# cherise215/advchain

Hardware: AMD Instinct MI355X
Metric: augmented images/sec (N adv steps, chain=noise+bias+morph+affine) (higher is better)
Workload: dtype f32

## Files before the change

advchain_amd/_lib.py:

```python
import ctypes
import os
from ctypes import c_char_p, c_float, c_int, c_int64, c_void_p

_HERE = os.path.dirname(os.path.abspath(__file__))
LIB_PATH = os.path.join(_HERE, "csrc", "libadvchain_hip.so")

_P, _I, _L, _F = c_void_p, c_int, c_int64, c_float

PROTOTYPES = {
    "advchain_version": (_I, []),
    "advchain_last_error": (c_char_p, []),
    "advchain_set_deterministic": (None, [_I]),
    "advchain_get_deterministic": (_I, []),
    "advchain_grid_sample_fwd": (_I, [_P, _P, _P, _L, _L, _I, _P, _P, _I, _I, _I, _P]),
    "advchain_grid_sample_fwd_ride": (_I, [_P, _P, _P, _P, _P, _L, _L, _I, _P, _P, _I, _I, _I, _I, _P]),
    "advchain_scatter_workspace": (_L, [_L, _I, _P]),
    "advchain_grid_sample_bwd": (_I, [_P, _P, _P, _P, _P, _P, _L, _L, _I, _P, _P, _I, _I, _I, _I, _P]),
    "advchain_compose_self_fwd": (_I, [_P, _P, _P, _L, _I, _P, _I, _P, _P]),
    "advchain_compose_self_bwd": (_I, [_P, _P, _P, _P, _I, _I, _L, _I, _P, _P]),
    "advchain_affine_warp_fwd": (_I, [_P, _P, _P, _L, _L, _I, _P, _I, _I, _P]),
    "advchain_affine_warp_fwd_ride": (_I, [_P, _P, _P, _P, _P, _L, _L, _I, _P, _I, _I, _I, _P]),
    "advchain_affine_warp_bwd_workspace": (_L, [_L, _I, _P]),
    "advchain_affine_warp_bwd": (_I, [_P, _P, _P, _P, _P, _P, _L, _L, _I, _P, _I, _I, _P]),
    "advchain_affine_theta_fwd": (_I, [_P, _P, _F, _P, _P, _L, _I, _P]),
    "advchain_affine_theta_bwd": (_I, [_P, _P, _F, _P, _P, _P, _L, _I, _P]),
    "advchain_tp_interp_fwd": (_I, [_P, _P, _P, _P, _P, _P, _P, _L, _L, _I, _I, _F, _P, _P, _P]),
    "advchain_tp_interp_fwd_smoothed_pair": (_I, [_P, _P, _P, _P, _P, _P, _P, _P, _L, _L, _I, _F, _P, _P, _F, _P]),
    "advchain_band_reduce_axis": (_I, [_P, _P, _P, _P, _P, _P, _P, _P, _I, _L, _L, _F, _P]),
    "advchain_band_reduce_rows_dense": (_I, [_P, _P, _P, _P, _P, _L, _L, _L, _L, _F, _P]),
    "advchain_bias_field_fwd": (_I, [_P, _P, _P, _P, _P, _P, _P, _P, _P, _L, _L, _F, _I, _F, _P]),
    "advchain_bias_field_bwd": (_I, [_P, _P, _P, _P, _P, _P, _P, _P, _P, _P, _L, _L, _F, _I, _F, _P]),
    "advchain_gauss_axis": (_I, [_P, _P, _P, _L, _L, _I, _P, _I, _P, _I, _I, _F, _P]),
    "advchain_gauss_axis_generic": (_I, [_P, _P, _L, _I, _P, _I, _P, _I, _F, _P]),
    "advchain_max_displacement": (_I, [_P, _P, _L, _I, _P, _P]),
    "advchain_grid_sample_bicubic2d_fwd": (_I, [_P, _P, _P, _L, _L, _P, _P, _I, _P]),
    "advchain_grid_sample_bicubic2d_bwd": (_I, [_P, _P, _P, _P, _P, _L, _L, _P, _P, _I, _P]),
    "advchain_affine_grid2d_fwd": (_I, [_P, _P, _L, _P, _P]),
    "advchain_affine_grid2d_bwd_workspace": (_L, [_L, _P]),
    "advchain_affine_grid2d_bwd": (_I, [_P, _P, _P, _L, _P, _P]),
    "advchain_slot_rows_max": (_I, [_P, _P, _L, _L, _I, _P]),
    "advchain_demons_compose_pair_fwd": (_I, [_P, _P, _P, _P, _P, _P, _P, _P, _P, _P, _P, _P, _P, _L, _I, _I, _P, _P, _F, _F, _I, _P]),
    "advchain_demons_compose_pair_bwd": (_I, [_P, _P, _P, _P, _P, _P, _P, _P, _P, _P, _P, _P, _P, _P, _P, _P, _P, _L, _P, _P, _P, _L,
                                              _I, _I, _P, _F, _F, _P]),
    "advchain_bounds_check": (_I, [_P, _P, _P, _L, _P, _P]),
    "advchain_expo_chain_fused_levels": (_I, [_L, _I, _P, _I, _P]),
    "advchain_expo_chain_fwd": (_I, [_P, _P, _P, _L, _I, _P, _I, _P, _P, _P, _P]),
# ... 132 lines not shown
```

advchain_amd/csrc/error.cpp:

```cpp
#include <string.h>

#include <atomic>

static thread_local char g_last_error[512] = "";

extern "C" void advchain_set_error_(const char* msg) {
  strncpy(g_last_error, msg ? msg : "", sizeof(g_last_error) - 1);
  g_last_error[sizeof(g_last_error) - 1] = 0;
}

extern "C" const char* advchain_last_error(void) { return g_last_error; }

static std::atomic<int> g_deterministic{0};
extern "C" void advchain_set_deterministic(int on) { g_deterministic.store(on ? 1 : 0, std::memory_order_relaxed); }
extern "C" int advchain_get_deterministic(void) { return g_deterministic.load(std::memory_order_relaxed); }

extern "C" int advchain_version(void) { return 130; }
```

advchain_amd/csrc/sampler.hip:

```cpp
#include <stdlib.h>
#include "sampler_common.h"
#include "affine_geo.h"

namespace advchain {

template <int UNR>
__device__ __forceinline__ void load_str(const float* __restrict__ p, int n, float (&r)[UNR]) {
#pragma unroll
  for (int k = 0; k < UNR; ++k) r[k] = p[(k < n ? k : 0) * kBlock];
#pragma unroll
  for (int k = 0; k < UNR; ++k) r[k] = k < n ? r[k] : 0.f;
}
template <int UNR>
__device__ __forceinline__ void store_str(float* __restrict__ p, int n, const float (&r)[UNR]) {
#pragma unroll
  for (int k = 0; k < UNR; ++k)
    if (k < n) p[k * kBlock] = r[k];
}
__device__ __forceinline__ int active_count(int64_t v0, int64_t total, int unr) {
  if (v0 >= total) return 0;
  const int64_t left = (total - v0 + kBlock - 1) / kBlock;
  return left < unr ? (int)left : unr;
}

// ... 620 lines not shown
  const int row = blockIdx.x;
  const int k = blockIdx.y;
  __shared__ float smem[4];
  float s[1] = {0.f};
  for (int b = threadIdx.x; b < nb; b += blockDim.x) s[0] += partial[((int64_t)row * nb + b) * K + k];
  block_sum<1>(s, smem);
  if (threadIdx.x == 0) out[(int64_t)row * K + k] = s[0];
}

}

using namespace advchain;

int advchain_scatter_tiled_launch(bool self, const float* gout, const float* in, const float* grid, float* gin,
                                  float* ggrid, int64_t N, int64_t C, int ndim, Dims d, int padding, int clamp_grid,
                                  int32_t* workspace, int chain, int halo, hipStream_t st);

int advchain_self_adjoint_gather_launch(const float* gout, const float* phi, float* gphi, int64_t N, int ndim, Dims d,
                                        int32_t* workspace, int chain, int halo, hipStream_t st);

int advchain_warp_adjoint_gather_launch(const float* gout, const float* in, const float* grid, float* gin, float* ggrid,
                                        int64_t N, int64_t C, int ndim, Dims d, int padding, int clamp_grid,
                                        int32_t* workspace, int halo, hipStream_t st);

int advchain_scatter_march_launch(bool self, const float* gout, const float* in, const float* grid, float* gin, float* ggrid,
                                  int64_t N, int64_t C, Dims d, int padding, int clamp_grid, int H, int32_t* workspace,
                                  hipStream_t st);

int advchain_scatter_window_launch(bool self, const float* gout, const float* in, const float* grid, float* gin,
                                   float* ggrid, int64_t N, int64_t C, int ndim, Dims d, int padding, int clamp_grid,
                                   int halo, int32_t* workspace, hipStream_t st, int32_t* det_ws);
int advchain_scatter_rows2d_launch(bool self, const float* gout, const float* in, const float* grid, float* gin, float* ggrid,
                                   int64_t N, int64_t C, Dims d, int padding, int clamp_grid, int H, int32_t* workspace,
                                   hipStream_t st, int rm_flags = 0);
bool advchain_scatter_rows2d_takes(bool self, int64_t C, Dims d, int padding, int H, int64_t N);

bool advchain_affine_box_fwd_launch(const float* in, const float* theta, float* out, int64_t N, int64_t C, int ndim, Dims d,
                                    hipStream_t st, const float* ride_in = nullptr, float* ride_out = nullptr,
                                    int ride_nonzero = 0);
int advchain_affine_box_tiles(int ndim, Dims d);
int advchain_affine_box_gtheta_launch(const float* gout, const float* in, const float* theta, float* gpart, int64_t N,
                                      int64_t C, int ndim, Dims d, int max_blocks, hipStream_t st, float* tilemax, float* geo = nullptr, int* mode = nullptr);
bool advchain_affine_box_gin_launch(const float* gout, const float* theta, const float* geo, const int* mode, float* gin,
                                    int64_t N, int64_t C, int ndim, Dims d, hipStream_t st, const float* tilemax);

int advchain_expo_fused_fwd2d_launch(const float* phi0, float* fields, int64_t N, advchain::Dims d, int k, int halos,
                                     float* disp_rows, float* fail_flag, hipStream_t stream, bool query = false);
int advchain_adjoint_fused2d_launch(const float* gk, const float* phi0, const float* fields, float* g0, int64_t N, advchain::Dims d,
                                    int k, int32_t* workspace, hipStream_t st);
int advchain_sample_tiled_launch(bool self, const float* in, const float* grid, float* out, const float* phi0,
                                 int64_t N, int64_t C, int ndim, Dims d, int padding, int clamp_grid, int final_mode,
                                 int halo, float* disp_out, hipStream_t st, int disp_hint);

static inline bool use_unroll(int64_t voxels, int ndim) {
  static const bool force1 = false;
  static const bool force4 = false;
  if (force4) return true;
  return !force1 && ndim == 2 && voxels >= 4 * kBlock;
}

#define DISPATCH_PAD(PADV, ...)                                            \
  switch (PADV) {                                                          \
    case PAD_ZEROS: { constexpr int PAD = PAD_ZEROS; __VA_ARGS__; } break; \
    case PAD_BORDER: { constexpr int PAD = PAD_BORDER; __VA_ARGS__; } break; \
    default: { constexpr int PAD = PAD_REFLECTION; __VA_ARGS__; } break;   \
  }

// ... 167 lines not shown
  ADVCHAIN_CHECK_ARG(final_mode == 0 || (final_mode == 1 && phi0), "compose_self_fwd: final_mode 1 needs phi0");
  ADVCHAIN_CHECK_ARG(N >= 0 && N < 65536, "compose_self_fwd: bad N");
  if (N == 0) return ADVCHAIN_OK;
  const Dims d = make_dims(ndim, dims);
  const int64_t V = d.voxels();
  ADVCHAIN_CHECK_ARG(V < (1ll << 31), "compose_self_fwd: per-sample volume too large");
  {
    const int rc = advchain_sample_tiled_launch(true, phi, nullptr, out, phi0, N, ndim, ndim, d, PAD_BORDER, 0,
                                                final_mode, 0, disp_out, (hipStream_t)stream, disp_hint);
    if (rc != ADVCHAIN_ERR_UNSUPPORTED) return rc;
  }
  const bool vec4 = use_unroll(V, ndim);
  hipStream_t st = (hipStream_t)stream;
  static const bool unr2 = true && true;
  if (unr2 && vec4 && ndim == 2) {
    dim3 g2(advchain_blocks(V, kBlock * 2), (unsigned)N);
    hipLaunchKernelGGL((k_compose_self_fwd<2, 2>), g2, dim3(kBlock), 0, st, phi, out, phi0, d, final_mode, disp_out);
    ADVCHAIN_LAUNCH_CHECK();
    return ADVCHAIN_OK;
  }
  dim3 g(advchain_blocks(V, kBlock * (vec4 ? 4 : 1)), (unsigned)N), b(kBlock);
  if (ndim == 3) {
    if (vec4) hipLaunchKernelGGL((k_compose_self_fwd<3, 4>), g, b, 0, st, phi, out, phi0, d, final_mode, disp_out);
    else hipLaunchKernelGGL((k_compose_self_fwd<3, 1>), g, b, 0, st, phi, out, phi0, d, final_mode, disp_out);
  } else {
    if (vec4) hipLaunchKernelGGL((k_compose_self_fwd<2, 4>), g, b, 0, st, phi, out, phi0, d, final_mode, disp_out);
    else hipLaunchKernelGGL((k_compose_self_fwd<2, 1>), g, b, 0, st, phi, out, phi0, d, final_mode, disp_out);
  }
  ADVCHAIN_LAUNCH_CHECK();
  return ADVCHAIN_OK;
}

static int compose_self_bwd_impl(const float* grad_out, const float* phi, float* grad_phi, int32_t* workspace, int chain,
                                 int halo, int64_t N, int ndim, const int64_t* dims, void* stream, int rm_flags);

int advchain_compose_self_bwd(const float* grad_out, const float* phi, float* grad_phi, int32_t* workspace, int chain,
                              int halo, int64_t N, int ndim, const int64_t* dims, void* stream) {
  return compose_self_bwd_impl(grad_out, phi, grad_phi, workspace, chain, halo, N, ndim, dims, stream, 0);
}

static int compose_self_bwd_impl(const float* grad_out, const float* phi, float* grad_phi, int32_t* workspace, int chain,
                                 int halo, int64_t N, int ndim, const int64_t* dims, void* stream, int rm_flags) {
  ADVCHAIN_CHECK_ARG(grad_out && phi && grad_phi, "compose_self_bwd: null pointer");
  ADVCHAIN_CHECK_ARG(dims_ok(ndim, dims), "compose_self_bwd: bad dims");
  ADVCHAIN_CHECK_ARG(N >= 0 && N < 65536, "compose_self_bwd: bad N");
  if (N == 0) return ADVCHAIN_OK;
  const Dims d = make_dims(ndim, dims);
  const int64_t V = d.voxels();
  ADVCHAIN_CHECK_ARG(V < (1ll << 31), "compose_self_bwd: per-sample volume too large");
  if (workspace) {
    if (ndim == 2 && halo <= -2) {
      const int rr = advchain_scatter_rows2d_launch(true, grad_out, phi, phi, grad_phi, nullptr, N, ndim, d, PAD_BORDER, 0, -halo,
                                                    workspace, (hipStream_t)stream, rm_flags);
      if (rr != ADVCHAIN_ERR_UNSUPPORTED) return rr;
    }
    const int rc = advchain_self_adjoint_gather_launch(grad_out, phi, grad_phi, N, ndim, d, workspace, chain, halo,
                                                       (hipStream_t)stream);
    if (rc != ADVCHAIN_ERR_UNSUPPORTED) return rc;
    if (ndim == 3 && halo <= -2) {
      const int rm = advchain_scatter_march_launch(true, grad_out, phi, phi, grad_phi, nullptr, N, ndim, d, PAD_BORDER, 0, -halo,
                                                   workspace, (hipStream_t)stream);
      if (rm != ADVCHAIN_ERR_UNSUPPORTED) return rm;
    }
    const int rw = advchain_scatter_window_launch(true, grad_out, phi, phi, grad_phi, nullptr, N, ndim, ndim, d, PAD_BORDER,
                                                  0, halo, workspace, (hipStream_t)stream, workspace);
    if (rw != ADVCHAIN_ERR_UNSUPPORTED) return rw;
    return advchain_scatter_tiled_launch(true, grad_out, phi, phi, grad_phi, nullptr, N, ndim, ndim, d, PAD_BORDER, 0,
                                         workspace, chain, halo < 0 ? -halo : halo, (hipStream_t)stream);
  }
  const bool vec4 = use_unroll(V, ndim);
  dim3 g(advchain_blocks(V, kBlock * (vec4 ? 4 : 1)), (unsigned)N), b(kBlock);
  hipStream_t st = (hipStream_t)stream;
  if (ndim == 3) {
    if (vec4) hipLaunchKernelGGL((k_compose_self_bwd<3, 4>), g, b, 0, st, grad_out, phi, grad_phi, d);
    else hipLaunchKernelGGL((k_compose_self_bwd<3, 1>), g, b, 0, st, grad_out, phi, grad_phi, d);
  } else {
    if (vec4) hipLaunchKernelGGL((k_compose_self_bwd<2, 4>), g, b, 0, st, grad_out, phi, grad_phi, d);
    else hipLaunchKernelGGL((k_compose_self_bwd<2, 1>), g, b, 0, st, grad_out, phi, grad_phi, d);
  }
  ADVCHAIN_LAUNCH_CHECK();
  return ADVCHAIN_OK;
}

int advchain_affine_warp_fwd(const float* in, const float* theta, float* out, int64_t N, int64_t C, int ndim,
                             const int64_t* dims, int interp, int padding, void* stream) {
  ADVCHAIN_CHECK_ARG(in && theta && out, "affine_warp_fwd: null pointer");
// ... 128 lines not shown
    }
  }
  if (fused) src = fields + (int64_t)(fused - 1) * F;
  for (int m = fused; m + 1 < n; ++m) {
    float* dst = fields + (int64_t)m * F;
    const int rc = advchain_compose_self_fwd(src, dst, nullptr, N, ndim, dims, hints ? (hints[m] & 0xff) << 8 : 0,
                                             disp_rows ? disp_rows + (int64_t)(m + 1) * kDispSlots : nullptr, stream);
    if (rc != ADVCHAIN_OK) return rc;
    src = dst;
  }
  return advchain_compose_self_fwd(src, pos, phi0, N, ndim, dims, 1 | (hints ? (hints[n - 1] & 0xff) << 8 : 0),
                                   disp_rows ? disp_rows + (int64_t)n * kDispSlots : nullptr, stream);
}

int advchain_expo_chain_bwd(const float* grad_pos, const float* phi0, const float* fields, float* grad_phi0, float* scratch,
                            int32_t* workspace, const int32_t* halos, int64_t N, int ndim, const int64_t* dims, int n,
                            void* stream) {
  ADVCHAIN_CHECK_ARG(grad_pos && phi0 && grad_phi0 && n >= 1 && n <= 64 && (n == 1 || (fields && scratch)) && halos,
                     "expo_chain_bwd: null pointer / bad n");
  ADVCHAIN_CHECK_ARG(dims_ok(ndim, dims), "expo_chain_bwd: bad dims");
  ADVCHAIN_CHECK_ARG(grad_phi0 != scratch && grad_pos != grad_phi0 && grad_pos != scratch, "expo_chain_bwd: aliased buffers");
  const int64_t F = N * ndim * make_dims(ndim, dims).voxels();
  int kf = 0;
  if (ndim == 2 && workspace && n >= 2) {
    while (kf < n && kf < 4 && halos[n - 1 - kf] == -1) ++kf;
    if (kf < 2) kf = 0;
  }
  const float* g = grad_pos;
  const Dims dd = make_dims(ndim, dims);
  static const bool no_handover = getenv("ADVCHAIN_NO_ROWMAX_HANDOVER") != nullptr;
  auto rows = [&](int i) {
    return !no_handover && ndim == 2 && workspace && i >= 0 && i < n - kf && halos[i] <= -2 && advchain_scatter_rows2d_takes(true, 2, dd, PAD_BORDER, -halos[i], N);
  };
  for (int i = 0; i < n - kf; ++i) {
    const int m = n - 1 - i;
    const float* phi = m == 0 ? phi0 : fields + (int64_t)(m - 1) * F;
    float* out = ((m - kf) % 2 == 0) ? (kf ? scratch : grad_phi0) : (kf ? grad_phi0 : scratch);
    const int rm = rows(i) ? ((rows(i - 1) ? 1 : 0) | (rows(i + 1) ? 2 : 0) | ((i & 1) ? 4 : 0)) : 0;
    const int rc = compose_self_bwd_impl(g, phi, out, workspace, i > 0 ? 1 : 0, halos[i], N, ndim, dims, stream, rm);
    if (rc != ADVCHAIN_OK) return rc;
    g = out;
  }
  if (kf) {
    const int rf = advchain_adjoint_fused2d_launch(g, phi0, fields, grad_phi0, N, make_dims(ndim, dims), kf, workspace,
                                                   (hipStream_t)stream);
    if (rf == ADVCHAIN_ERR_UNSUPPORTED) {
      for (int m = kf - 1; m >= 0; --m) {
        const float* phi = m == 0 ? phi0 : fields + (int64_t)(m - 1) * F;
        float* out = (m % 2 == 0) ? grad_phi0 : scratch;
        if (out == g) {
          float* other = out == grad_phi0 ? scratch : grad_phi0;
          (void)hipMemcpyAsync(other, g, sizeof(float) * F, hipMemcpyDeviceToDevice, (hipStream_t)stream);
          g = other;
        }
        const int rc = advchain_compose_self_bwd(g, phi, out, workspace, (n - 1 - m) > 0 ? 1 : 0, halos[n - 1 - m], N, ndim, dims, stream);
        if (rc != ADVCHAIN_OK) return rc;
        g = out;
      }
    } else if (rf != ADVCHAIN_OK) {
      return rf;
    } else {
      ADVCHAIN_LAUNCH_CHECK();
    }
  }
  return ADVCHAIN_OK;
}

int64_t advchain_affine_warp_bwd_workspace(int64_t N, int ndim, const int64_t* dims) {
  if (!dims_ok(ndim, dims)) return -1;
  const Dims d = make_dims(ndim, dims);
  return N * (int64_t)affine_grid_blocks(d) * ndim * (ndim + 1) + N * (kGeoFloats + 1) + N * (int64_t)advchain_affine_box_tiles(ndim, d);
}
// ... 86 lines not shown
```

advchain_amd/csrc/scatter_march.hip:

```cpp
#include <stdlib.h>
#include "sampler_common.h"

namespace advchain {

__device__ __forceinline__ float ld_off(const float* __restrict__ base, unsigned byte_off) {
  return *reinterpret_cast<const float*>(reinterpret_cast<const char*>(base) + byte_off);
}
__device__ __forceinline__ void st_off(float* __restrict__ base, unsigned byte_off, float v) {
  *reinterpret_cast<float*>(reinterpret_cast<char*>(base) + byte_off) = v;
}

template <int DIM, int PAD>
__device__ __forceinline__ void coord_path_values(const float (&vl)[8], float go, const Taps<DIM, PAD>& t, float& ax, float& ay,
                                                  float& az);

template <int DIM, int PAD>
__device__ __forceinline__ void coord_path_diff(const float* __restrict__ in, float go, const Taps<DIM, PAD>& t, const Dims& d,
                                                float& ax, float& ay, float& az) {
  const CornerOffsets<DIM, PAD> o(t, d);
  float vl[8];
  o.load(in, vl);
  coord_path_values<DIM, PAD>(vl, go, t, ax, ay, az);
}

template <int DIM, int PAD>
__device__ __forceinline__ void coord_path_values(const float (&vl)[8], float go, const Taps<DIM, PAD>& t, float& ax, float& ay,
                                                  float& az) {
  float v[2][2][2];
#pragma unroll
  for (int cz = 0; cz < (DIM == 3 ? 2 : 1); ++cz)
#pragma unroll
    for (int cy = 0; cy < 2; ++cy)
#pragma unroll
      for (int cx = 0; cx < 2; ++cx) v[cz][cy][cx] = vl[(cz * 2 + cy) * 2 + cx];
#pragma unroll
  for (int cz = 0; cz < (DIM == 3 ? 2 : 1); ++cz)
#pragma unroll
    for (int cy = 0; cy < 2; ++cy)
#pragma unroll
      for (int cx = 0; cx < 2; ++cx) v[cz][cy][cx] = t.ok(cz, cy, cx) ? v[cz][cy][cx] : 0.f;
  if (DIM == 3) {
    float sx = 0.f, sy = 0.f;
#pragma unroll
    for (int cz = 0; cz < 2; ++cz) {
      sx = fmaf(t.wz(cz), fmaf(t.y.w1, v[cz][1][1] - v[cz][1][0], t.y.w0 * (v[cz][0][1] - v[cz][0][0])), sx);
      sy = fmaf(t.wz(cz), fmaf(t.x.w1, v[cz][1][1] - v[cz][0][1], t.x.w0 * (v[cz][1][0] - v[cz][0][0])), sy);
    }
    float sz = 0.f;
#pragma unroll
    for (int cy = 0; cy < 2; ++cy)
      sz = fmaf(t.wy(cy), fmaf(t.x.w1, v[1][cy][1] - v[0][cy][1], t.x.w0 * (v[1][cy][0] - v[0][cy][0])), sz);
    ax = fmaf(go, sx, ax);
    ay = fmaf(go, sy, ay);
    az = fmaf(go, sz, az);
  } else {
    ax = fmaf(go, fmaf(t.y.w1, v[0][1][1] - v[0][1][0], t.y.w0 * (v[0][0][1] - v[0][0][0])), ax);
    ay = fmaf(go, fmaf(t.x.w1, v[0][1][1] - v[0][0][1], t.x.w0 * (v[0][1][0] - v[0][0][0])), ay);
  }
}

__device__ __forceinline__ int march_fix_bits(int H) { return H <= 2 ? 23 : (H == 3 ? 22 : (H == 4 ? 21 : 18)); }

template <int C>
__global__ void __launch_bounds__(kBlock) k_march_rowmax(const float* __restrict__ x, float* __restrict__ rowmax, Dims d, int rows_per_n,
                                                                int ctot = C) {
  constexpr int RW = 4;
  const int lane = threadIdx.x & 63;
  const int row0 = (blockIdx.x * (kBlock / 64) + (threadIdx.x >> 6)) * RW;
  const int n = blockIdx.y;
  if (row0 >= rows_per_n) return;
  const int V = (int)d.voxels();
  const float* p = x + (int64_t)n * ctot * V;
  float m[RW];
  bool bad[RW];
#pragma unroll
  for (int r = 0; r < RW; ++r) { m[r] = 0.f; bad[r] = false; }
  for (int xx = lane; xx < d.s2; xx += 64) {
    float v[RW][C];
#pragma unroll
    for (int r = 0; r < RW; ++r) {
      const int row = min(row0 + r, rows_per_n - 1);
#pragma unroll
      for (int c = 0; c < C; ++c) v[r][c] = p[(int64_t)c * V + (int64_t)row * d.s2 + xx];
    }
#pragma unroll
    for (int r = 0; r < RW; ++r)
#pragma unroll
      for (int c = 0; c < C; ++c) {
        m[r] = fmaxf(m[r], fabsf(v[r][c]));
        bad[r] = bad[r] || !(fabsf(v[r][c]) <= 3.0e38f);
      }
  }
#pragma unroll
  for (int r = 0; r < RW; ++r) {
#pragma unroll
    for (int o = 32; o > 0; o >>= 1) m[r] = fmaxf(m[r], __shfl_xor(m[r], o, 64));
    if (__ballot(bad[r]) != 0) m[r] = __int_as_float(0x7f800000);
  }
  if (lane < RW && row0 + lane < rows_per_n) {
    float mine = m[0];
#pragma unroll
    for (int r = 1; r < RW; ++r) mine = lane == r ? m[r] : mine;
    rowmax[(int64_t)n * rows_per_n + row0 + lane] = mine;
  }
}

template <int C>
__global__ void __launch_bounds__(kBlock) k_march_rowmax64(const float* __restrict__ x, float* __restrict__ rowmax, int rows_per_n, int ctot) {
  constexpr int U = 4;
  const int lane = threadIdx.x & 63;
  const int row0 = (blockIdx.x * (kBlock / 64) + (threadIdx.x >> 6)) * (4 * U) + (lane >> 4);
  const int n = blockIdx.y;
  if (row0 - (lane >> 4) >= rows_per_n) return;
  const int64_t V = (int64_t)rows_per_n * 64;
  const float* p = x + (int64_t)n * ctot * V + (lane & 15) * 4;
  float4 v[U][C];
#pragma unroll
  for (int u = 0; u < U; ++u) {
    const int row = min(row0 + 4 * u, rows_per_n - 1);
#pragma unroll
    for (int c = 0; c < C; ++c) v[u][c] = *reinterpret_cast<const float4*>(p + (int64_t)c * V + (int64_t)row * 64);
  }
#pragma unroll
  for (int u = 0; u < U; ++u) {
    float m = 0.f;
    bool bad = false;
#pragma unroll
    for (int c = 0; c < C; ++c) {
      const float q = fmaxf(fmaxf(fabsf(v[u][c].x), fabsf(v[u][c].y)), fmaxf(fabsf(v[u][c].z), fabsf(v[u][c].w)));
      m = fmaxf(m, q);
      bad = bad || !(fabsf(v[u][c].x) <= 3.0e38f) || !(fabsf(v[u][c].y) <= 3.0e38f) || !(fabsf(v[u][c].z) <= 3.0e38f) ||
            !(fabsf(v[u][c].w) <= 3.0e38f);
    }
    if (bad) m = __int_as_float(0x7f800000);
#pragma unroll
    for (int o = 8; o > 0; o >>= 1) m = fmaxf(m, __shfl_xor(m, o, 64));
    const int row = row0 + 4 * u;
// ... 771 lines not shown
      int4* cell = reinterpret_cast<int4*>(acc + (((zt % NS) + NS) % NS) * (TY * 64) + row * 64 + 4 * q);
      const int4 c = *cell;
      *cell = make_int4(0, 0, 0, 0);
      if (uy < d.s1 && 4 * q < d.s2) {
        fprev = make_float4(fix_out((float)c.x, fs), fix_out((float)c.y, fs), fix_out((float)c.z, fs), fix_out((float)c.w, fs));
        fo_prev = (unsigned)((zt * d.s1 + uy) * d.s2 + 4 * q) * 4u;
        *reinterpret_cast<float4*>(reinterpret_cast<char*>(ginn) + fo_prev) = fprev;
      }
    }
    cur ^= 1;
  };
  for (int zp = za - H; zp < zb + H; zp += 2) {
    step(zp, rowA, inA, rowB, inB);
    if (zp + 1 < zb + H) step(zp + 1, rowB, inB, rowA, inA);
  }
  if (GG && have_prev) {
    st_off(ggn, so_prev, gg_prev[0]);
    st_off(ggn + V, so_prev, gg_prev[1]);
    st_off(ggn + (int64_t)2 * V, so_prev, gg_prev[2]);
  }
}

#ifndef ADVCHAIN_ROWS2D_FLAT
#define ADVCHAIN_ROWS2D_FLAT 1
#endif
__device__ __forceinline__ int rows2d_fix_bits(int H) {
  return H <= 2 ? 25 : (H <= 4 ? 24 : (H <= 8 ? 22 : (H <= 16 ? 20 : 18)));
}

template <int PAD, int C, bool SELF, bool GG>
__global__ void __launch_bounds__(512)
k_scatter_rows2d(const float* __restrict__ gout, const float* __restrict__ in, const float* __restrict__ grid,
                 float* __restrict__ gin, float* __restrict__ ggrid, Dims d, int TY, int H, int clamp_grid,
                 int32_t* __restrict__ ws, const float* __restrict__ rowmax_in, float* __restrict__ rowmax_next) {
  extern __shared__ int acc[];
  __shared__ int rmax[64];
  constexpr int NWV = 8;
  const int W = d.s2, V = d.s1 * d.s2;
  const int n = blockIdx.y;
  const int lane = threadIdx.x & 63, wave = threadIdx.x >> 6;
  const int y0 = blockIdx.x * TY, yend = min(y0 + TY, d.s1);
  const int nseg = (W + 63) >> 6;
  const float* gn = grid + (int64_t)n * 2 * V;
  const float* gon = gout + (int64_t)n * C * V;
  const float* inn = in + (int64_t)n * C * V;
  float* ginn = gin + (int64_t)n * C * V;
  const int ya = max(y0 - H, 0), yb = min(y0 + TY + H, d.s1);
  __shared__ float wmax[NWV];
  {
    const float* rowmax = rowmax_in + (int64_t)n * d.s1;
    float m = 0.f;
    for (int y = ya + (int)threadIdx.x; y < yb; y += NWV * 64) m = fmaxf(m, rowmax[y]);
    if (threadIdx.x < 64) rmax[threadIdx.x] = 0;
#pragma unroll
    for (int o = 32; o > 0; o >>= 1) m = fmaxf(m, __shfl_xor(m, o, 64));
    if (lane == 0) wmax[wave] = m;
  }
  for (int i = threadIdx.x; i < C * TY * W; i += NWV * 64) acc[i] = 0;
  if (SELF && blockIdx.x == 0 && blockIdx.y == 0 && threadIdx.x == 0) ws[3] = -1;
  __syncthreads();
  float gmax = wmax[0];
#pragma unroll
  for (int w = 1; w < NWV; ++w) gmax = fmaxf(gmax, wmax[w]);
  const FixScale fs = fix_scale(gmax, rows2d_fix_bits(H));
  float scale_p, inv_p;
  const bool plain = fix_plain(fs, scale_p, inv_p);
  auto body = [&](auto plain_tag) {
  constexpr bool PLAIN = decltype(plain_tag)::value;

  constexpr int U = 2;
  constexpr int MAXO = 8;
  const int oitems = (yend - y0) * nseg;
  const float inv_nseg = 1.f / (float)nseg;
  auto item_row = [&](int it) { return (int)(((float)it + 0.5f) * inv_nseg); };
  float ggv[MAXO][2];
  auto visit = [&](int ys, int xs0, bool own, float (&g)[2], const float (&go)[C], float (&gg)[2]) {
    const bool xin = xs0 < W;
    bool pass[2] = {true, true};
    if (clamp_grid) {
#pragma unroll
      for (int a = 0; a < 2; ++a) { pass[a] = g[a] >= -1.f && g[a] <= 1.f; g[a] = clamp_unit(g[a]); }
    }
    Taps<2, PAD> t;
    t.y = make_tap<PAD>(g[1], d.s1);
    const bool any = __ballot(xin && t.y.i0 + 1 >= y0 && t.y.i0 < yend) != 0;
    if (!any && !(own && (SELF || GG))) return;
    t.x = make_tap<PAD>(g[0], d.s2);
    t.z.i0 = 0; t.z.w0 = 1.f; t.z.w1 = 0.f; t.z.mult = 0.f; t.z.v0 = true; t.z.v1 = false;
    float vl[C][8];
    if (own && (SELF || GG)) {
      const CornerOffsets<2, PAD> o(t, d);
#pragma unroll
      for (int c = 0; c < C; ++c) o.load(inn + (int64_t)c * V, vl[c]);
    }
    if (any) {
      float gs[C];
#pragma unroll
      for (int c = 0; c < C; ++c) gs[c] = PLAIN ? go[c] : fix_in(go[c], fs);
      if constexpr (ADVCHAIN_ROWS2D_FLAT && SELF) {
      const int ownr = __mul24(min(max(ys - y0, 0), TY - 1), W), ownc = min(xs0, W - 1);
      int rowc[2], colc[2];
      float wxm[2], wym[2];
#pragma unroll
      for (int cx = 0; cx < 2; ++cx) {
        const bool ok = xin && (cx ? t.x.v1 : t.x.v0);
        wxm[cx] = ok ? (cx ? t.x.w1 : t.x.w0) * (PLAIN ? scale_p : fs.mul) : 0.f;
        colc[cx] = ok ? t.x.i0 + cx : ownc;
// ... 32 lines not shown
    }
    if (own && (SELF || GG)) {
      float ax = 0.f, ay = 0.f, az = 0.f;
#pragma unroll
      for (int c = 0; c < C; ++c) coord_path_values<2, PAD>(vl[c], go[c], t, ax, ay, az);
      gg[0] = pass[0] ? t.x.mult * ax : 0.f;
      gg[1] = pass[1] ? t.y.mult * ay : 0.f;
    }
    (void)ys;
  };
#pragma unroll
  for (int k0 = 0; k0 < MAXO; k0 += U) {
    float g[U][2], go[U][C];
    int xs[U], ys[U];
#pragma unroll
    for (int u = 0; u < U; ++u) {
      ggv[k0 + u][0] = ggv[k0 + u][1] = 0.f;
      const int it = min(wave + (k0 + u) * NWV, max(oitems - 1, 0));
      const int r = item_row(it);
      ys[u] = y0 + r;
      xs[u] = (it - r * nseg) * 64 + lane;
      const int s = ys[u] * W + min(xs[u], W - 1);
      g[u][0] = gn[s];
      g[u][1] = gn[V + s];
#pragma unroll
      for (int c = 0; c < C; ++c) go[u][c] = gon[(int64_t)c * V + s];
    }
#pragma unroll
    for (int u = 0; u < U; ++u) {
      if (wave + (k0 + u) * NWV >= oitems) continue;
      visit(ys[u], xs[u], true, g[u], go[u], ggv[k0 + u]);
    }
  }
  const int hlo = y0 - ya, hitems = (hlo + (yb - yend)) * nseg;
  for (int it0 = wave * U; it0 < hitems; it0 += NWV * U) {
    float g[U][2], go[U][C];
    int xs[U], ys[U];
#pragma unroll
    for (int u = 0; u < U; ++u) {
      const int it = min(it0 + u, hitems - 1);
      const int r = item_row(it);
      ys[u] = r < hlo ? ya + r : yend + (r - hlo);
      xs[u] = (it - r * nseg) * 64 + lane;
      const int s = ys[u] * W + min(xs[u], W - 1);
      g[u][0] = gn[s];
      g[u][1] = gn[V + s];
#pragma unroll
      for (int c = 0; c < C; ++c) go[u][c] = gon[(int64_t)c * V + s];
    }
#pragma unroll
    for (int u = 0; u < U; ++u) {
      if (it0 + u >= hitems) continue;
      float dummy[2];
      visit(ys[u], xs[u], false, g[u], go[u], dummy);
    }
  }
  __syncthreads();
#pragma unroll
  for (int k = 0; k < MAXO; ++k) {
    const int it = wave + k * NWV;
    if (it >= oitems) continue;
    const int r = item_row(it);
    const int x = (it - r * nseg) * 64 + lane;
    const bool on = x < W;
    const int s = (y0 + r) * W + min(x, W - 1);
    float v[C];
#pragma unroll
    for (int c = 0; c < C; ++c) {
      const float q = (float)acc[(c * TY + r) * W + min(x, W - 1)];
      if (PLAIN) v[c] = SELF ? fmaf(q, inv_p, ggv[k][c < 2 ? c : 0]) : q * inv_p;
      else v[c] = SELF ? fix_out_add(q, ggv[k][c < 2 ? c : 0], fs) : fix_out(q, fs);
    }
    if (!SELF && GG) {
      float* gq = ggrid + (int64_t)n * 2 * V + s;
      if (on) { gq[0] = ggv[k][0]; gq[V] = ggv[k][1]; }
    }
    if (on) {
#pragma unroll
      for (int c = 0; c < C; ++c) ginn[(int64_t)c * V + s] = v[c];
    }
    if (rowmax_next) {
      float m = 0.f;
      bool bad = false;
#pragma unroll
      for (int c = 0; c < C; ++c) {
// ... 4 lines not shown
      for (int o = 32; o > 0; o >>= 1) m = fmaxf(m, __shfl_xor(m, o, 64));
      if (__ballot(bad) != 0) m = __int_as_float(0x7f800000);
      if (lane == 0) atomicMax(&rmax[r], __float_as_int(m));
    }
  }
  if (rowmax_next) {
    __syncthreads();
    if ((int)threadIdx.x < yend - y0) rowmax_next[(int64_t)n * d.s1 + y0 + threadIdx.x] = __int_as_float(rmax[threadIdx.x]);
  }
  };
  if (plain) body(std::true_type{});
  else body(std::false_type{});
}

}

using namespace advchain;

static int rows2d_tile(bool self, int64_t C, const Dims& d, int padding, int H, int64_t N) {
  static const bool off = getenv("ADVCHAIN_NO_SCATTER_ROWS2D") != nullptr;
  const int hmin = (self && N * ((d.s1 + 15) / 16) >= 512) ? 2 : 3;
  if (off || padding == PAD_REFLECTION || H < hmin || H > (self ? 32 : 16) || d.s0 != 1) return 0;
  if (d.s2 < 16 || d.s2 > 512 || d.voxels() * 4 >= (1ll << 31)) return 0;
  if (self ? C != 2 : (C != 1 && C != 4)) return 0;
  const int nseg = (d.s2 + 63) / 64;
  int TY = H >= 8 ? 32 : 16;
  static const size_t lds_cap = 49152;
  while (TY > 4 && ((size_t)C * TY * d.s2 * 4 > lds_cap || TY * nseg > 64)) TY >>= 1;
  if ((size_t)C * TY * d.s2 * sizeof(int) > 65536 - 64 || TY * nseg > 64) return 0;
  return TY;
}
bool advchain_scatter_rows2d_takes(bool self, int64_t C, Dims d, int padding, int H, int64_t N) { return rows2d_tile(self, C, d, padding, H, N) > 0; }

int advchain_scatter_rows2d_launch(bool self, const float* gout, const float* in, const float* grid, float* gin, float* ggrid,
                                   int64_t N, int64_t C, Dims d, int padding, int clamp_grid, int H, int32_t* workspace,
                                   hipStream_t st, int rm_flags) {
  const int TY = (workspace && gin) ? rows2d_tile(self, C, d, padding, H, N) : 0;
  if (TY == 0) return ADVCHAIN_ERR_UNSUPPORTED;
  const size_t lds = (size_t)C * TY * d.s2 * sizeof(int);
  float* rm_a = reinterpret_cast<float*>(workspace + 4);
  float* rm_b = rm_a + N * d.s1;
  float* rm_in = (rm_flags & 4) ? rm_b : rm_a;
  float* rm_next = (rm_flags & 2) ? ((rm_flags & 4) ? rm_a : rm_b) : nullptr;
  if (!(rm_flags & 1)) {
    dim3 rg((unsigned)((d.s1 + kBlock / 16 - 1) / (kBlock / 16)), (unsigned)N);
    if (C == 1) hipLaunchKernelGGL(k_march_rowmax<1>, rg, dim3(kBlock), 0, st, gout, rm_in, d, d.s1);
    else if (C == 2) hipLaunchKernelGGL(k_march_rowmax<2>, rg, dim3(kBlock), 0, st, gout, rm_in, d, d.s1);
    else hipLaunchKernelGGL(k_march_rowmax<4>, rg, dim3(kBlock), 0, st, gout, rm_in, d, d.s1);
  }
  dim3 g((unsigned)((d.s1 + TY - 1) / TY), (unsigned)N), b(512);
  const bool gg = ggrid != nullptr;
#define GO(PAD_, C_, SELF_, GG_) \
  hipLaunchKernelGGL((k_scatter_rows2d<PAD_, C_, SELF_, GG_>), g, b, lds, st, gout, in, grid, gin, ggrid, d, TY, H, clamp_grid, workspace, rm_in, rm_next)
#define GO_PAD(C_, GG_) do { if (padding == PAD_BORDER) GO(PAD_BORDER, C_, false, GG_); else GO(PAD_ZEROS, C_, false, GG_); } while (0)
  if (self) GO(PAD_BORDER, 2, true, false);
  else if (C == 1) { if (gg) GO_PAD(1, true); else GO_PAD(1, false); }
  else { if (gg) GO_PAD(4, true); else GO_PAD(4, false); }
#undef GO_PAD
#undef GO
  ADVCHAIN_LAUNCH_CHECK();
  return ADVCHAIN_OK;
}

int advchain_scatter_march_launch(bool self, const float* gout, const float* in, const float* grid, float* gin, float* ggrid,
                                  int64_t N, int64_t C, Dims d, int padding, int clamp_grid, int H, int32_t* workspace,
                                  hipStream_t st) {
  static const bool off = getenv("ADVCHAIN_NO_SCATTER_MARCH") != nullptr;
  static const int hmax = 8;
  if (off || !workspace || !gin || padding == PAD_REFLECTION || H < 2 || H > hmax || H > 8) return ADVCHAIN_ERR_UNSUPPORTED;
  if (d.s2 > 1024 || d.s2 < 8 || d.s0 < 2 || d.voxels() * 4 >= (1ll << 31)) return ADVCHAIN_ERR_UNSUPPORTED;
  const int nseg = d.s2 <= 64 ? 1 : (int)((d.s2 + (64 - 2 * H) - 1) / (64 - 2 * H));
  if (self ? C != 3 : (C != 1 && C != 4)) return ADVCHAIN_ERR_UNSUPPORTED;
  if (H > 4 && C == 1 && N * d.voxels() < (6ll << 20)) return ADVCHAIN_ERR_UNSUPPORTED;
  if (H > 4) {
    const int NSb = 2 * H + 3, TYb = 8;
    const size_t ldsb = (size_t)NSb * TYb * 64 * sizeof(int);
    const int n1b = (d.s1 + TYb - 1) / TYb;
    int zcb = d.s0;
    while (zcb > 32 && N * n1b * nseg * ((d.s0 + zcb - 1) / zcb) < 512) zcb = (zcb + 1) / 2;
    const int n0b = (d.s0 + zcb - 1) / zcb;
    dim3 gb((unsigned)(n1b * n0b * nseg), (unsigned)N), bb(512);
    const int rows = (int)(d.s0 * d.s1);
    dim3 rg((unsigned)((rows + kBlock / 16 - 1) / (kBlock / 16)), (unsigned)N);
    float* rowmax = reinterpret_cast<float*>(workspace + 4);
    const bool ggb = ggrid != nullptr;
#define GOB(PAD_, SELF_, GG_, CT_) \
// ... 108 lines not shown
```

advchain_amd/ops.py:

```python
import ctypes
import functools
import os

import numpy as np
import torch

from . import _lib
from .bands import gaussian_weights_1d

_INTERP = {"bilinear": 0, "trilinear": 0, "linear": 0, "nearest": 1, "bicubic": 2}
_PAD = {"zeros": 0, "border": 1, "reflection": 2}
_GAUSS9 = _lib.float_array(gaussian_weights_1d(1.0))
_GAUSS9_CACHE = {}


GENERIC_MAX_TAPS = 129


def gauss9(sigma, taps=None):
    sigma = float(sigma)
    if taps is None:
        taps = 2 * int(4 * sigma + 0.5) + 1
    taps = int(taps)
    if sigma == 1.0 and taps == 9:
# ... 115 lines not shown


def raw_grid_sample_fwd_ride(inp, grid, ride, interp, padding, clamp_grid, nonzero, disp_hint=None):
    N, C = inp.shape[:2]
    nd = inp.dim() - 2
    odims = tuple(grid.shape[2:])
    out = torch.empty((N, C) + odims, device=inp.device, dtype=torch.float32)
    rout = torch.empty((N, 1) + odims, device=inp.device, dtype=torch.float32)
    _lib.check(_lib.load().advchain_grid_sample_fwd_ride(_ptr(inp), _ptr(grid), _ptr(out), _ptr(ride), _ptr(rout), N, C, nd,
                                                         _lib.dims_array(inp.shape[2:]), _lib.dims_array(odims), interp, padding,
                                                         int(clamp_grid) | _hint_bits(disp_hint), int(bool(nonzero)), _stream()),
               "grid_sample_fwd_ride")
    return out, rout


DISP_SLOTS = 4096
ADAPTIVE_HALO = os.environ.get("ADVCHAIN_NO_ADAPTIVE_HALO") is None
PAIR_FIELDS = os.environ.get("ADVCHAIN_NO_PAIR_FIELDS") is None
TILED_SCATTER = True
FUSED_LOSS = True
WIDE_LOSS_MIN_K = 17
FUSE_2D = True
COMPOSITE = True
RIDE_MASK = True
RIDE_INTERPS = ("bilinear", "trilinear", "linear", "nearest")


def set_deterministic(on):
    _lib.load().advchain_set_deterministic(1 if on else 0)


def is_deterministic():
    return bool(_lib.load().advchain_get_deterministic())


def _scatter_workspace(N, dims, device):
    n = _lib.load().advchain_scatter_workspace(N, len(dims), _lib.dims_array(dims))
    return torch.empty(n, device=device, dtype=torch.int32)


def raw_grid_sample_bwd(gout, inp, grid, interp, padding, clamp_grid, need_gin, need_ggrid, halo=0):
    N, C = inp.shape[:2]
    nd = inp.dim() - 2
    tiled = TILED_SCATTER and need_gin
    ws = _scatter_workspace(N, inp.shape[2:], inp.device) if tiled else None
    gin = (torch.empty_like(inp) if tiled else torch.zeros_like(inp)) if need_gin else None
    ggrid = torch.empty_like(grid) if need_ggrid else None
    _lib.check(_lib.load().advchain_grid_sample_bwd(_ptr(gout), _ptr(inp), _ptr(grid), _ptr(gin), _ptr(ggrid), _ptr(ws),
                                                    N, C, nd, _lib.dims_array(inp.shape[2:]),
                                                    _lib.dims_array(grid.shape[2:]), interp, padding, int(clamp_grid),
                                                    int(halo), _stream()), "grid_sample_bwd")
    return gin, ggrid


def raw_compose_self_fwd(phi, phi0=None, final_mode=0, disp_out=None, disp_hint=None):
    N = phi.shape[0]
    nd = phi.dim() - 2
    out = torch.empty_like(phi)
    _lib.check(_lib.load().advchain_compose_self_fwd(_ptr(phi), _ptr(out), _ptr(phi0), N, nd,
                                                     _lib.dims_array(phi.shape[2:]), final_mode | _hint_bits(disp_hint), _ptr(disp_out),
                                                     _stream()), "compose_self_fwd")
    return out


def raw_compose_self_bwd(gout, phi, ws=None, chain=False, halo=0):
    N = phi.shape[0]
# ... 1567 lines not shown
```

include/advchain_hip.h:

```cpp
#ifndef ADVCHAIN_HIP_H_
#define ADVCHAIN_HIP_H_

#include <stdint.h>

#ifdef __cplusplus
extern "C" {
#endif

#define ADVCHAIN_INTERP_LINEAR 0
#define ADVCHAIN_INTERP_NEAREST 1
#define ADVCHAIN_INTERP_BICUBIC 2
#define ADVCHAIN_PAD_ZEROS 0
#define ADVCHAIN_PAD_BORDER 1
#define ADVCHAIN_PAD_REFLECTION 2

int advchain_version(void);
const char* advchain_last_error(void);

void advchain_set_deterministic(int on);
int advchain_get_deterministic(void);

int advchain_grid_sample_fwd(const float* in, const float* grid, float* out, int64_t N, int64_t C, int ndim,
                             const int64_t* in_dims, const int64_t* out_dims, int interp, int padding,
                             int clamp_grid, void* stream);
int advchain_grid_sample_fwd_ride(const float* in, const float* grid, float* out, const float* ride_in, float* ride_out,
                                  int64_t N, int64_t C, int ndim, const int64_t* in_dims, const int64_t* out_dims,
                                  int interp, int padding, int clamp_grid, int flags, void* stream);
int64_t advchain_scatter_workspace(int64_t N, int ndim, const int64_t* dims);
int advchain_grid_sample_bwd(const float* grad_out, const float* in, const float* grid, float* grad_in,
                             float* grad_grid, int32_t* workspace, int64_t N, int64_t C, int ndim,
                             const int64_t* in_dims, const int64_t* out_dims, int interp, int padding, int clamp_grid,
                             int halo, void* stream);

#define ADVCHAIN_DISP_SLOTS 4096
int advchain_compose_self_fwd(const float* phi, float* out, const float* phi0, int64_t N, int ndim,
                              const int64_t* dims, int final_mode, float* disp_out, void* stream);
int advchain_compose_self_bwd(const float* grad_out, const float* phi, float* grad_phi, int32_t* workspace, int chain,
                              int halo, int64_t N, int ndim, const int64_t* dims, void* stream);
int advchain_expo_chain_fused_levels(int64_t N, int ndim, const int64_t* dims, int n, const int32_t* hints);
int advchain_expo_chain_fwd(const float* phi0, float* fields, float* pos, int64_t N, int ndim, const int64_t* dims, int n,
                            float* disp_rows, const int32_t* hints, float* fuse_flag, void* stream);
int advchain_expo_chain_bwd(const float* grad_pos, const float* phi0, const float* fields, float* grad_phi0, float* scratch,
                            int32_t* workspace, const int32_t* halos, int64_t N, int ndim, const int64_t* dims, int n,
                            void* stream);
int advchain_demons_compose_pair_fwd(const float* vel, float* s1, float* phi0, float* fields, float* pos, float* q,
                                     float* disp, float* rows_max, const int32_t* itab, const float* ftab,
                                     const int64_t* S3, const int64_t* g3, const int64_t* B3, int64_t N, int ndim, int n,
                                     const int32_t* hints, const float* weights9_host, float scale, float inv, int fuse,
                                     void* stream);
int advchain_demons_compose_pair_bwd(const float* gq_lo, const float* gq_hi, const float* pos, const float* phi0,
                                     const float* fields, float* gpos, float* g, float* scratch, int32_t* ws, float* t1,
                                     float* gs1, float* gvel, const int32_t* halos, const int32_t* itab, const float* ftab,
                                     const float* wd, const int32_t* wlo, int64_t WB, const int64_t* S3, const int64_t* g3,
// ... 148 lines not shown
```

Baseline: 3965.

## Prune halo rows in rows2d scatter using precomputed per-segment reach tables

Adds a prepass kernel that, for every level of a consecutive run of rows2d scatter launches, records the min/max source row each 64-wide segment of the grid touches. It is fused with the existing rowmax computation. The scatter kernel then uses these tables to build a compacted list of halo items whose scatter can land in its own tile, and skips the rest. This cuts redundant halo visits, at the cost of an extra prepass, extra LDS and a block-wide sync. The feature is enabled by default and has a runtime toggle.

```diff
diff --git a/advchain_amd/_lib.py b/advchain_amd/_lib.py
--- a/advchain_amd/_lib.py
+++ b/advchain_amd/_lib.py
@@ -12,6 +12,8 @@
     "advchain_last_error": (c_char_p, []),
     "advchain_set_deterministic": (None, [_I]),
     "advchain_get_deterministic": (_I, []),
+    "advchain_set_rows2d_reach": (None, [_I]),
+    "advchain_get_rows2d_reach": (_I, []),
     "advchain_grid_sample_fwd": (_I, [_P, _P, _P, _L, _L, _I, _P, _P, _I, _I, _I, _P]),
     "advchain_grid_sample_fwd_ride": (_I, [_P, _P, _P, _P, _P, _L, _L, _I, _P, _P, _I, _I, _I, _I, _P]),
     "advchain_scatter_workspace": (_L, [_L, _I, _P]),
diff --git a/advchain_amd/csrc/error.cpp b/advchain_amd/csrc/error.cpp
--- a/advchain_amd/csrc/error.cpp
+++ b/advchain_amd/csrc/error.cpp
@@ -15,4 +15,8 @@
 extern "C" void advchain_set_deterministic(int on) { g_deterministic.store(on ? 1 : 0, std::memory_order_relaxed); }
 extern "C" int advchain_get_deterministic(void) { return g_deterministic.load(std::memory_order_relaxed); }
 
+static std::atomic<int> g_rows2d_reach{1};
+extern "C" void advchain_set_rows2d_reach(int on) { g_rows2d_reach.store(on ? 1 : 0, std::memory_order_relaxed); }
+extern "C" int advchain_get_rows2d_reach(void) { return g_rows2d_reach.load(std::memory_order_relaxed); }
+
 extern "C" int advchain_version(void) { return 130; }
diff --git a/advchain_amd/csrc/sampler.hip b/advchain_amd/csrc/sampler.hip
--- a/advchain_amd/csrc/sampler.hip
+++ b/advchain_amd/csrc/sampler.hip
@@ -676,7 +676,8 @@
                                    int halo, int32_t* workspace, hipStream_t st, int32_t* det_ws);
 int advchain_scatter_rows2d_launch(bool self, const float* gout, const float* in, const float* grid, float* gin, float* ggrid,
                                    int64_t N, int64_t C, Dims d, int padding, int clamp_grid, int H, int32_t* workspace,
-                                   hipStream_t st, int rm_flags = 0);
+                                   hipStream_t st, int rm_flags = 0, const float* const* run_grids = nullptr, int run_len = 1,
+                                   int run_pos = 0);
 bool advchain_scatter_rows2d_takes(bool self, int64_t C, Dims d, int padding, int H, int64_t N);
 
 bool advchain_affine_box_fwd_launch(const float* in, const float* theta, float* out, int64_t N, int64_t C, int ndim, Dims d,
@@ -910,7 +911,8 @@
 }
 
 static int compose_self_bwd_impl(const float* grad_out, const float* phi, float* grad_phi, int32_t* workspace, int chain,
-                                 int halo, int64_t N, int ndim, const int64_t* dims, void* stream, int rm_flags);
+                                 int halo, int64_t N, int ndim, const int64_t* dims, void* stream, int rm_flags,
+                                 const float* const* run_grids = nullptr, int run_len = 1, int run_pos = 0);
 
 int advchain_compose_self_bwd(const float* grad_out, const float* phi, float* grad_phi, int32_t* workspace, int chain,
                               int halo, int64_t N, int ndim, const int64_t* dims, void* stream) {
@@ -918,7 +920,8 @@
 }
 
 static int compose_self_bwd_impl(const float* grad_out, const float* phi, float* grad_phi, int32_t* workspace, int chain,
-                                 int halo, int64_t N, int ndim, const int64_t* dims, void* stream, int rm_flags) {
+                                 int halo, int64_t N, int ndim, const int64_t* dims, void* stream, int rm_flags,
+                                 const float* const* run_grids, int run_len, int run_pos) {
   ADVCHAIN_CHECK_ARG(grad_out && phi && grad_phi, "compose_self_bwd: null pointer");
   ADVCHAIN_CHECK_ARG(dims_ok(ndim, dims), "compose_self_bwd: bad dims");
   ADVCHAIN_CHECK_ARG(N >= 0 && N < 65536, "compose_self_bwd: bad N");
@@ -929,7 +932,7 @@
   if (workspace) {
     if (ndim == 2 && halo <= -2) {
       const int rr = advchain_scatter_rows2d_launch(true, grad_out, phi, phi, grad_phi, nullptr, N, ndim, d, PAD_BORDER, 0, -halo,
-                                                    workspace, (hipStream_t)stream, rm_flags);
+                                                    workspace, (hipStream_t)stream, rm_flags, run_grids, run_len, run_pos);
       if (rr != ADVCHAIN_ERR_UNSUPPORTED) return rr;
     }
     const int rc = advchain_self_adjoint_gather_launch(grad_out, phi, grad_phi, N, ndim, d, workspace, chain, halo,
@@ -1124,12 +1127,21 @@
   auto rows = [&](int i) {
     return !no_handover && ndim == 2 && workspace && i >= 0 && i < n - kf && halos[i] <= -2 && advchain_scatter_rows2d_takes(true, 2, dd, PAD_BORDER, -halos[i], N);
   };
+  auto level_phi = [&](int i) { return n - 1 - i == 0 ? phi0 : fields + (int64_t)(n - 2 - i) * F; };
+  const float* run_grids[64];
+  int run_first = 0, run_len = 1;
   for (int i = 0; i < n - kf; ++i) {
     const int m = n - 1 - i;
-    const float* phi = m == 0 ? phi0 : fields + (int64_t)(m - 1) * F;
+    const float* phi = level_phi(i);
     float* out = ((m - kf) % 2 == 0) ? (kf ? scratch : grad_phi0) : (kf ? grad_phi0 : scratch);
     const int rm = rows(i) ? ((rows(i - 1) ? 1 : 0) | (rows(i + 1) ? 2 : 0) | ((i & 1) ? 4 : 0)) : 0;
-    const int rc = compose_self_bwd_impl(g, phi, out, workspace, i > 0 ? 1 : 0, halos[i], N, ndim, dims, stream, rm);
+    if (!(rm & 1)) {
+      run_first = i;
+      run_grids[0] = phi;
+      for (run_len = 1; rows(i) && rows(i + run_len); ++run_len) run_grids[run_len] = level_phi(i + run_len);
+    }
+    const int rc = compose_self_bwd_impl(g, phi, out, workspace, i > 0 ? 1 : 0, halos[i], N, ndim, dims, stream, rm, run_grids,
+                                         run_len, i - run_first);
     if (rc != ADVCHAIN_OK) return rc;
     g = out;
   }
diff --git a/advchain_amd/csrc/scatter_march.hip b/advchain_amd/csrc/scatter_march.hip
--- a/advchain_amd/csrc/scatter_march.hip
+++ b/advchain_amd/csrc/scatter_march.hip
@@ -1,4 +1,7 @@
 #include <stdlib.h>
+
+#include <algorithm>
+
 #include "sampler_common.h"
 
 namespace advchain {
@@ -61,14 +64,12 @@
 
 __device__ __forceinline__ int march_fix_bits(int H) { return H <= 2 ? 23 : (H == 3 ? 22 : (H == 4 ? 21 : 18)); }
 
+constexpr int kRowmaxRows = 4;
 template <int C>
-__global__ void __launch_bounds__(kBlock) k_march_rowmax(const float* __restrict__ x, float* __restrict__ rowmax, Dims d, int rows_per_n,
-                                                                int ctot = C) {
-  constexpr int RW = 4;
+__device__ __forceinline__ void march_rowmax_rows(const float* __restrict__ x, float* __restrict__ rowmax, const Dims& d, int rows_per_n,
+                                                  int ctot, int row0, int n) {
+  constexpr int RW = kRowmaxRows;
   const int lane = threadIdx.x & 63;
-  const int row0 = (blockIdx.x * (kBlock / 64) + (threadIdx.x >> 6)) * RW;
-  const int n = blockIdx.y;
-  if (row0 >= rows_per_n) return;
   const int V = (int)d.voxels();
   const float* p = x + (int64_t)n * ctot * V;
   float m[RW];
@@ -103,6 +104,48 @@
     for (int r = 1; r < RW; ++r) mine = lane == r ? m[r] : mine;
     rowmax[(int64_t)n * rows_per_n + row0 + lane] = mine;
   }
+}
+template <int C>
+__global__ void __launch_bounds__(kBlock) k_march_rowmax(const float* __restrict__ x, float* __restrict__ rowmax, Dims d, int rows_per_n,
+                                                                int ctot = C) {
+  const int row0 = (blockIdx.x * (kBlock / 64) + (threadIdx.x >> 6)) * kRowmaxRows;
+  if (row0 >= rows_per_n) return;
+  march_rowmax_rows<C>(x, rowmax, d, rows_per_n, ctot, row0, blockIdx.y);
+}
+
+constexpr int kReachLevels = 16;
+struct ReachGrids { const float* g[kReachLevels]; };
+__device__ __forceinline__ int reach_limit(int i0, int S) { return min(max(i0, -2), S) + 2; }
+
+template <int C, int PAD>
+__global__ void __launch_bounds__(kBlock) k_rows2d_prepass(const float* __restrict__ x, float* __restrict__ rowmax, Dims d, ReachGrids grids,
+                                                           unsigned int* __restrict__ reach, int clamp_grid) {
+  constexpr int RW = kRowmaxRows;
+  const int lane = threadIdx.x & 63;
+  const int row0 = (blockIdx.x * (kBlock / 64) + (threadIdx.x >> 6)) * RW;
+  const int n = blockIdx.y, lev = blockIdx.z;
+  if (row0 >= d.s1) return;
+  const int W = d.s2, nseg = (W + 63) >> 6;
+  const float* gy = grids.g[lev] + ((int64_t)n * 2 + 1) * d.s1 * W;
+  unsigned int* tab = reach + ((int64_t)lev * gridDim.y + n) * d.s1 * nseg;
+  for (int seg = 0; seg < nseg; ++seg) {
+    const int xx = min(seg * 64 + lane, W - 1);
+    float v[RW];
+#pragma unroll
+    for (int r = 0; r < RW; ++r) v[r] = gy[(int64_t)min(row0 + r, d.s1 - 1) * W + xx];
+#pragma unroll
+    for (int r = 0; r < RW; ++r) {
+      const int i0 = reach_limit(make_tap<PAD>(clamp_grid ? clamp_unit(v[r]) : v[r], d.s1).i0, d.s1);
+      int lo = i0, hi = i0;
+#pragma unroll
+      for (int o = 32; o > 0; o >>= 1) {
+        lo = min(lo, __shfl_xor(lo, o, 64));
+        hi = max(hi, __shfl_xor(hi, o, 64));
+      }
+      if (lane == 0 && row0 + r < d.s1) tab[(row0 + r) * nseg + seg] = (unsigned)lo | ((unsigned)hi << 16);
+    }
+  }
+  if (lev == 0) march_rowmax_rows<C>(x, rowmax, d, d.s1, C, row0, n);
 }
 
 template <int C>
@@ -940,9 +983,12 @@
 __global__ void __launch_bounds__(512)
 k_scatter_rows2d(const float* __restrict__ gout, const float* __restrict__ in, const float* __restrict__ grid,
                  float* __restrict__ gin, float* __restrict__ ggrid, Dims d, int TY, int H, int clamp_grid,
-                 int32_t* __restrict__ ws, const float* __restrict__ rowmax_in, float* __restrict__ rowmax_next) {
+                 int32_t* __restrict__ ws, const float* __restrict__ rowmax_in, float* __restrict__ rowmax_next,
+                 const unsigned int* __restrict__ reach) {
   extern __shared__ int acc[];
   __shared__ int rmax[64];
+  __shared__ unsigned short hlist[512];
+  __shared__ int hcnt[8];
   constexpr int NWV = 8;
   const int W = d.s2, V = d.s1 * d.s2;
   const int n = blockIdx.y;
@@ -964,12 +1010,39 @@
     for (int o = 32; o > 0; o >>= 1) m = fmaxf(m, __shfl_xor(m, o, 64));
     if (lane == 0) wmax[wave] = m;
   }
+  const float inv_nseg = 1.f / (float)nseg;
+  auto item_row = [&](int it) { return (int)(((float)it + 0.5f) * inv_nseg); };
+  const int hlo = y0 - ya, hitems = (hlo + (yb - yend)) * nseg;
+  bool hreach = false;
+  int hcode = 0;
+  if ((int)threadIdx.x < hitems) {
+    const int r = item_row(threadIdx.x), seg = threadIdx.x - r * nseg;
+    const int ys = r < hlo ? ya + r : yend + (r - hlo);
+    hcode = (ys - ya) * 8 + seg;
+    hreach = true;
+    if (reach) {
+      const unsigned e = reach[((int64_t)n * d.s1 + ys) * nseg + seg];
+      hreach = (int)(e >> 16) - 2 + 1 >= y0 && (int)(e & 0xffffu) - 2 < yend;
+    }
+  }
+  const unsigned long long hballot = __ballot(hreach);
+  if (lane == 0) hcnt[wave] = __popcll(hballot);
   for (int i = threadIdx.x; i < C * TY * W; i += NWV * 64) acc[i] = 0;
   if (SELF && blockIdx.x == 0 && blockIdx.y == 0 && threadIdx.x == 0) ws[3] = -1;
   __syncthreads();
   float gmax = wmax[0];
 #pragma unroll
   for (int w = 1; w < NWV; ++w) gmax = fmaxf(gmax, wmax[w]);
+  int nreach = 0;
+  {
+    int before = 0;
+#pragma unroll
+    for (int w = 0; w < NWV; ++w) {
+      before += w < wave ? hcnt[w] : 0;
+      nreach += hcnt[w];
+    }
+    if (hreach) hlist[before + __popcll(hballot & ((1ull << lane) - 1ull))] = (unsigned short)hcode;
+  }
   const FixScale fs = fix_scale(gmax, rows2d_fix_bits(H));
   float scale_p, inv_p;
   const bool plain = fix_plain(fs, scale_p, inv_p);
@@ -979,8 +1052,6 @@
   constexpr int U = 2;
   constexpr int MAXO = 8;
   const int oitems = (yend - y0) * nseg;
-  const float inv_nseg = 1.f / (float)nseg;
-  auto item_row = [&](int it) { return (int)(((float)it + 0.5f) * inv_nseg); };
   float ggv[MAXO][2];
   auto visit = [&](int ys, int xs0, bool own, float (&g)[2], const float (&go)[C], float (&gg)[2]) {
     const bool xin = xs0 < W;
@@ -1079,16 +1150,15 @@
       visit(ys[u], xs[u], true, g[u], go[u], ggv[k0 + u]);
     }
   }
-  const int hlo = y0 - ya, hitems = (hlo + (yb - yend)) * nseg;
-  for (int it0 = wave * U; it0 < hitems; it0 += NWV * U) {
+  __syncthreads();
+  for (int it0 = wave * U; it0 < nreach; it0 += NWV * U) {
     float g[U][2], go[U][C];
     int xs[U], ys[U];
 #pragma unroll
     for (int u = 0; u < U; ++u) {
-      const int it = min(it0 + u, hitems - 1);
-      const int r = item_row(it);
-      ys[u] = r < hlo ? ya + r : yend + (r - hlo);
-      xs[u] = (it - r * nseg) * 64 + lane;
+      const int code = hlist[min(it0 + u, nreach - 1)];
+      ys[u] = ya + (code >> 3);
+      xs[u] = (code & 7) * 64 + lane;
       const int s = ys[u] * W + min(xs[u], W - 1);
       g[u][0] = gn[s];
       g[u][1] = gn[V + s];
@@ -1097,7 +1167,7 @@
     }
 #pragma unroll
     for (int u = 0; u < U; ++u) {
-      if (it0 + u >= hitems) continue;
+      if (it0 + u >= nreach) continue;
       float dummy[2];
       visit(ys[u], xs[u], false, g[u], go[u], dummy);
     }
@@ -1168,9 +1238,10 @@
 }
 bool advchain_scatter_rows2d_takes(bool self, int64_t C, Dims d, int padding, int H, int64_t N) { return rows2d_tile(self, C, d, padding, H, N) > 0; }
 
+extern "C" int advchain_get_rows2d_reach(void);
 int advchain_scatter_rows2d_launch(bool self, const float* gout, const float* in, const float* grid, float* gin, float* ggrid,
                                    int64_t N, int64_t C, Dims d, int padding, int clamp_grid, int H, int32_t* workspace,
-                                   hipStream_t st, int rm_flags) {
+                                   hipStream_t st, int rm_flags, const float* const* run_grids, int run_len, int run_pos) {
   const int TY = (workspace && gin) ? rows2d_tile(self, C, d, padding, H, N) : 0;
   if (TY == 0) return ADVCHAIN_ERR_UNSUPPORTED;
   const size_t lds = (size_t)C * TY * d.s2 * sizeof(int);
@@ -1178,7 +1249,24 @@
   float* rm_b = rm_a + N * d.s1;
   float* rm_in = (rm_flags & 4) ? rm_b : rm_a;
   float* rm_next = (rm_flags & 2) ? ((rm_flags & 4) ? rm_a : rm_b) : nullptr;
-  if (!(rm_flags & 1)) {
+  const int64_t slot = N * d.s1 * ((d.s2 + 63) / 64);
+  const int64_t slots = advchain_get_rows2d_reach() && d.s1 <= 65000 ? std::min<int64_t>(kReachLevels, (2 * N * (d.voxels() - d.s1)) / slot) : 0;
+  unsigned int* const tabs = reinterpret_cast<unsigned int*>(rm_a + 2 * N * d.s1);
+  if (!(rm_flags & 1)) run_pos = 0;
+  const unsigned int* reach = run_pos < slots ? tabs + run_pos * slot : nullptr;
+  if (!(rm_flags & 1) && slots > 0) {
+    ReachGrids rgs = {};
+    rgs.g[0] = grid;
+    int nlev = 1;
+    if (run_grids)
+      for (nlev = 0; nlev < run_len && nlev < slots; ++nlev) rgs.g[nlev] = run_grids[nlev];
+    dim3 rg((unsigned)((d.s1 + kBlock / 16 - 1) / (kBlock / 16)), (unsigned)N, (unsigned)nlev);
+#define PRE(C_, PAD_) hipLaunchKernelGGL((k_rows2d_prepass<C_, PAD_>), rg, dim3(kBlock), 0, st, gout, rm_in, d, rgs, tabs, clamp_grid)
+    if (C == 2) PRE(2, PAD_BORDER);
+    else if (C == 1) { if (padding == PAD_BORDER) PRE(1, PAD_BORDER); else PRE(1, PAD_ZEROS); }
+    else { if (padding == PAD_BORDER) PRE(4, PAD_BORDER); else PRE(4, PAD_ZEROS); }
+#undef PRE
+  } else if (!(rm_flags & 1)) {
     dim3 rg((unsigned)((d.s1 + kBlock / 16 - 1) / (kBlock / 16)), (unsigned)N);
     if (C == 1) hipLaunchKernelGGL(k_march_rowmax<1>, rg, dim3(kBlock), 0, st, gout, rm_in, d, d.s1);
     else if (C == 2) hipLaunchKernelGGL(k_march_rowmax<2>, rg, dim3(kBlock), 0, st, gout, rm_in, d, d.s1);
@@ -1187,7 +1275,7 @@
   dim3 g((unsigned)((d.s1 + TY - 1) / TY), (unsigned)N), b(512);
   const bool gg = ggrid != nullptr;
 #define GO(PAD_, C_, SELF_, GG_) \
-  hipLaunchKernelGGL((k_scatter_rows2d<PAD_, C_, SELF_, GG_>), g, b, lds, st, gout, in, grid, gin, ggrid, d, TY, H, clamp_grid, workspace, rm_in, rm_next)
+  hipLaunchKernelGGL((k_scatter_rows2d<PAD_, C_, SELF_, GG_>), g, b, lds, st, gout, in, grid, gin, ggrid, d, TY, H, clamp_grid, workspace, rm_in, rm_next, reach)
 #define GO_PAD(C_, GG_) do { if (padding == PAD_BORDER) GO(PAD_BORDER, C_, false, GG_); else GO(PAD_ZEROS, C_, false, GG_); } while (0)
   if (self) GO(PAD_BORDER, 2, true, false);
   else if (C == 1) { if (gg) GO_PAD(1, true); else GO_PAD(1, false); }
diff --git a/advchain_amd/ops.py b/advchain_amd/ops.py
--- a/advchain_amd/ops.py
+++ b/advchain_amd/ops.py
@@ -171,6 +171,14 @@
 
 def is_deterministic():
     return bool(_lib.load().advchain_get_deterministic())
+
+
+def set_rows2d_reach(on):
+    _lib.load().advchain_set_rows2d_reach(1 if on else 0)
+
+
+def rows2d_reach():
+    return bool(_lib.load().advchain_get_rows2d_reach())
 
 
 def _scatter_workspace(N, dims, device):
diff --git a/include/advchain_hip.h b/include/advchain_hip.h
--- a/include/advchain_hip.h
+++ b/include/advchain_hip.h
@@ -19,6 +19,9 @@
 
 void advchain_set_deterministic(int on);
 int advchain_get_deterministic(void);
+
+void advchain_set_rows2d_reach(int on);
+int advchain_get_rows2d_reach(void);
 
 int advchain_grid_sample_fwd(const float* in, const float* grid, float* out, int64_t N, int64_t C, int ndim,
                              const int64_t* in_dims, const int64_t* out_dims, int interp, int padding,
```

Result: slower. 3917 (-1.2%).
